# winddori2002/DEX-TTS

Hardware: AMD Instinct MI355X
Metric: mel-frames/s at n_timesteps=50, 80-ch mel (sampler only); RTF (higher is better)
Workload: dtype bf16; 1 GPU; gedex_b1: gedex_lj B=1/GPU T=512 n_timesteps=50 (BASELINE.json configs[1]); global_batch=1, frames=512, hipgraph=False, parallelism=1 GPU

## Files before the change

### dex_tts_amd/csrc/conv3x3_bf16.hip

```cpp
#include "kernels.h"
#include <cstdlib>
#include <cstdio>
#include "lp_util.h"
#include "kernels_lp.h"
#include "conv_gn.h"

namespace dex {
namespace DEX_LP_NS {

typedef float f32x16 __attribute__((ext_vector_type(16)));
typedef unsigned short u16;
typedef unsigned u32x4 __attribute__((ext_vector_type(4)));

__device__ __forceinline__ float cv_mish(float x) {
    const float e = __expf(fminf(x, 20.f));
    const float n = e * (e + 2.f);
    return x * (n * __builtin_amdgcn_rcpf(n + 2.f));
}

template <int NT, int COUT>
__device__ __forceinline__ void cv_epilogue(const Conv3P& p, f32x16 (&acc)[NT], int b, int ho, int w0, int nbase, int lane, int tid,
                                            long long* gnred) {
    const int i = lane & 31, hh = lane >> 5;
    constexpr int cpg = COUT / 8;
    if (p.gn_stats) { if (tid < 16) gnred[tid] = 0; __syncthreads(); }
    const bool full = ho < p.H && w0 + 32 <= p.W;
    const long ybase = (long)b * p.H * p.W * COUT + ((long)ho * p.W + w0 + 4 * hh) * COUT + nbase + i;
    float* yl = p.Y + ybase;
    u16* yh = reinterpret_cast<u16*>(p.Y) + ybase;
    const bool yb = p.y_bf16 != 0;
#pragma unroll
    for (int t = 0; t < NT; ++t) {
        const int n = nbase + t * 32 + i;
        const float bias = p.bias[n];
        float gs = 0.f, gss = 0.f;
        if (full && yb) {
            const bool odd = (lane & 1) != 0;
            u16* yp = yh + (odd ? 16 * COUT - 1 : 0) + t * 32;
#pragma unroll
            for (int r = 0; r < 16; ++r) { const float v = acc[t][r] + bias; gs += v; gss = fmaf(v, v, gss); }
#pragma unroll
            for (int j = 0; j < 8; ++j) {
                const float lo_r = acc[t][j] + bias, hi_r = acc[t][8 + j] + bias;
                const float recv = lane_xor1(odd ? lo_r : hi_r);
                const float mine = odd ? hi_r : lo_r;
                const unsigned pk = odd ? pack2_lp(recv, mine) : pack2_lp(mine, recv);
                *reinterpret_cast<unsigned*>(yp + ((j & 3) + 8 * (j >> 2)) * COUT) = pk;
            }
        } else if (full) {
            const bool odd = (lane & 1) != 0;
            float* yp = yl + (odd ? 16 * COUT - 1 : 0) + t * 32;
#pragma unroll
            for (int r = 0; r < 16; ++r) { const float v = acc[t][r] + bias; gs += v; gss = fmaf(v, v, gss); }
#pragma unroll
            for (int j = 0; j < 8; ++j) {
                const float lo_r = acc[t][j] + bias, hi_r = acc[t][8 + j] + bias;
                const float recv = lane_xor1(odd ? lo_r : hi_r);
                const float mine = odd ? hi_r : lo_r;
                *reinterpret_cast<float2*>(yp + ((j & 3) + 8 * (j >> 2)) * COUT) = odd ? make_float2(recv, mine) : make_float2(mine, recv);
            }
        } else {
#pragma unroll
            for (int r = 0; r < 16; ++r) {
                const int wo = w0 + (r & 3) + 8 * (r >> 2) + 4 * hh;
                const bool ok = ho < p.H && wo < p.W;
                const float v = acc[t][r] + bias;
                const float vs = ok ? v : 0.f;
                gs += vs; gss = fmaf(vs, vs, gss);
                if (ok) {
                    if (yb) yh[((r & 3) + 8 * (r >> 2)) * COUT + t * 32] = lp_bits(v);
                    else yl[((r & 3) + 8 * (r >> 2)) * COUT + t * 32] = v;
                }
            }
        }
        if (p.gn_stats) {
            for (int o = 1; o < cpg; o <<= 1) { gs += __shfl_xor(gs, o); gss += __shfl_xor(gss, o); }
            gs += __shfl_xor(gs, 32); gss += __shfl_xor(gss, 32);
            if (hh == 0 && (i & (cpg - 1)) == 0) {
                const double inv_n = 1.0 / ((double)p.H * p.W * cpg);
                gn_add(&gnred[(n / cpg) * 2], gn_fix(gs, inv_n)); gn_add(&gnred[(n / cpg) * 2 + 1], gn_fix(gss, inv_n));
            }
        }
    }
    if (p.gn_stats) {
        __syncthreads();
        if (tid < 16) {
            const long long v = gnred[tid];
            if (v != 0) {
                const int slot = (blockIdx.x + blockIdx.y * gridDim.x) % GN_SLOTS;
                gn_add(p.gn_stats + (((long)b * 8 + (tid >> 1)) * GN_SLOTS + slot) * 2 + (tid & 1), v);
            }
        }
    }
}

template <int NT, int COUT>
__device__ __forceinline__ void cv_res_store(const Conv3P& p, const f32x16 (&accr)[NT], int b, int ho, int w0, int nb, int lane) {
    const int i = lane & 31, hh = lane >> 5;
    float* yl = p.res_y + ((long)b * p.H * p.W + (long)ho * p.W + w0 + 4 * hh) * COUT + nb + i;
    const bool rfull = ho < p.H && w0 + 32 <= p.W;
    const bool odd = (lane & 1) != 0;
#pragma unroll
    for (int t = 0; t < NT; ++t) {
        const float bias = p.res_b[nb + t * 32 + i];
        if (rfull) {
            float* yp = yl + (odd ? 16 * COUT - 1 : 0) + t * 32;
#pragma unroll
            for (int j = 0; j < 8; ++j) {
                const float lo_r = accr[t][j] + bias, hi_r = accr[t][8 + j] + bias;
                const float recv = lane_xor1(odd ? lo_r : hi_r);
                const float mine = odd ? hi_r : lo_r;
                *reinterpret_cast<float2*>(yp + ((j & 3) + 8 * (j >> 2)) * COUT) = odd ? make_float2(recv, mine) : make_float2(mine, recv);
            }
        } else {
#pragma unroll
            for (int r = 0; r < 16; ++r) {
                const int wo = w0 + (r & 3) + 8 * (r >> 2) + 4 * hh;
                if (ho < p.H && wo < p.W) yl[((r & 3) + 8 * (r >> 2)) * COUT + t * 32] = accr[t][r] + bias;
            }
        }
    }
}

template <int CC, int COUT, int NSL, int TH, bool PRO2 = false, bool RES = false, bool XB = false, int NW = 4>
__global__ __launch_bounds__(64 * NW) void conv3x3_lp_kernel(const Conv3P p) {
    constexpr int PW = 34, PH = TH + 2;
    constexpr int LDP = CC + 8;
    constexpr int WN = NW / TH;
    constexpr int NTHR = 64 * NW;
    constexpr int NT = NSL / 32 / WN;
    constexpr int NSLICE = COUT / NSL;
    constexpr int ITEMS = PH * PW * (CC / 8);
    constexpr int NI = (ITEMS + NTHR - 1) / NTHR;
    constexpr int WITEMS = NSL * CC / 8;
    constexpr int WPT = (WITEMS + NTHR - 1) / NTHR;
    constexpr bool WFULL = WITEMS % NTHR == 0;
    constexpr int RING = CC == 128 ? (PRO2 ? 1 : 2) : 3;
    constexpr int NPASS = TH == 5 ? (CC == 128 ? (PRO2 ? 6 : 3) : (PRO2 ? 3 : XB ? 1 : 2))
                                  : CC == 128 ? (TH == 8 ? (PRO2 ? 8 : 4) : (PRO2 ? 5 : 2)) : (PRO2 ? 3 : 1);
    constexpr int NIP = (NI + NPASS - 1) / NPASS;
#ifdef DEX_LP_WSPLIT
    constexpr int NTAP = 18;
#else
    constexpr int NTAP = 9;
#endif
    static_assert(NT >= 1 && WPT >= 1 && NW % TH == 0 && NTHR % (CC / 8) == 0, "tile");
    extern __shared__ __attribute__((aligned(16))) u16 smem[];
    u16* patch = smem;
    u16* wbuf = smem + PH * PW * LDP;
    u16* rbuf = wbuf + 2 * NSL * LDP;
    __shared__ long long gnred[16];
    constexpr int COEF_N = (TH == 8) ? 128 : 256;
    __shared__ __attribute__((aligned(16))) float coef[3][COEF_N];

    const int tid = threadIdx.x, lane = tid & 63, wave = tid >> 6;
    const int i = lane & 31, hh = lane >> 5;
    const int wrow = wave % TH, wcol = wave / TH;
#ifdef DEX_TIMING
    long long tk[8] = {0, 0, 0, 0, 0, 0, 0, 0};
    const long long tk0 = __builtin_readcyclecounter();
    long long tlast = tk0;
#define CSTAMP(k) do { const long long now_ = __builtin_readcyclecounter(); tk[k] += now_ - tlast; tlast = now_; } while (0)
#else
#define CSTAMP(k) do {} while (0)
#endif
    const int xs = p.skip_dead ? (int)((blockIdx.x + blockIdx.y + blockIdx.z) % gridDim.x) : (int)blockIdx.x;
    const int w0 = xs * 32, h0 = blockIdx.y * TH;
    const int b = blockIdx.z / NSLICE, slice = blockIdx.z % NSLICE;
    const int step = p.step + b * p.row_bstride;
    const float* X = p.X + (long)b * p.H * p.W * p.ldx + p.x_coff;
    const u16* Xh = reinterpret_cast<const u16*>(p.X) + (long)b * p.H * p.W * p.ldx + p.x_coff;
    const float* mrow = p.mask + (long)b * p.mask_bstride;
    const int K = 9 * p.Cin;
    const u16* Wg = reinterpret_cast<const u16*>(p.Wbf) + (long)slice * NSL * K;
    const bool pro = p.pro_stats != nullptr;
    if constexpr (!PRO2) {
        if (p.skip_dead) {
            const int wi = w0 - 1 + (lane < 34 ? lane : 33);
            const float mv = (unsigned)wi < (unsigned)p.W ? mrow[wi * p.mask_ws] : 0.f;
            if (__builtin_amdgcn_ballot_w64(mv != 0.f) == 0) {
                f32x16 zacc[NT];
#pragma unroll
                for (int t = 0; t < NT; ++t)
#pragma unroll
                    for (int r = 0; r < 16; ++r) zacc[t][r] = 0.f;
                if constexpr (RES) cv_res_store<NT, COUT>(p, zacc, b, h0 + wrow, w0, slice * NSL + wcol * NT * 32, lane);
                cv_epilogue<NT, COUT>(p, zacc, b, h0 + wrow, w0, slice * NSL + wcol * NT * 32, lane, tid, gnred);
                return;
            }
        }
    }

    f32x16 acc[NT];
#pragma unroll
    for (int t = 0; t < NT; ++t)
#pragma unroll
        for (int r = 0; r < 16; ++r) acc[t][r] = 0.f;

    f32x16 accr[RES ? NT : 1];
    if constexpr (RES) {
#pragma unroll
        for (int t = 0; t < NT; ++t)
#pragma unroll
            for (int r = 0; r < 16; ++r) accr[t][r] = 0.f;
    }
    int wofs[WPT], wlds[WPT];
    bool wok[WPT];
#pragma unroll
    for (int j = 0; j < WPT; ++j) {
        const int it = tid + NTHR * j;
        const int n = it / (CC / 8), c8 = (it % (CC / 8)) * 8;
        wofs[j] = n * K + c8;
        wlds[j] = n * LDP + c8;
        wok[j] = WFULL || it < WITEMS;
    }
    const int pc8 = (tid % (CC / 8)) * 8;

    CvGnLoads gnl{};
    if (pro) gnl = cv_gn_issue(p, b, tid, step);
    const int nchunk = p.Cin / CC;
    for (int ch = 0; ch < nchunk; ++ch) {
        const int cbase = ch * CC;
        u32x4 w0r[WPT], wr[RING][WPT], rwr[RES ? WPT : 1];
#ifdef DEX_LP_WSPLIT
        u32x4 rwl[RES ? WPT : 1];
#define WS_TAPOFS(t) ((long)((t) % 9) * p.Cin + ((t) >= 9 ? p.w_lo_off : 0L))
#else
#define WS_TAPOFS(t) ((long)(t) * p.Cin)
#endif
        float4 sc0, sc1, sh0, sh1, t0, t1;
#pragma unroll
        for (int ps = 0; ps < NPASS; ++ps) {
            float4 pf0[NIP], pf1[XB ? 1 : NIP], rf0[PRO2 ? NIP : 1], rf1[PRO2 ? NIP : 1];
            float pmk[NIP];
            bool pin[NIP];
#pragma unroll
            for (int q = 0; q < NIP; ++q) {
                const int it = min(tid + NTHR * (ps * NIP + q), ITEMS - 1);
                const int px = it / (CC / 8);
                const int pw = px % PW, ph = px / PW;
                const int hi = h0 + ph - 1, wi = w0 + pw - 1;
                const bool inb = (unsigned)hi < (unsigned)p.H && (unsigned)wi < (unsigned)p.W;
                const int hc = inb ? hi : 0, wc = inb ? wi : 0;
                if constexpr (XB) {
                    pf0[q] = *reinterpret_cast<const float4*>(Xh + ((long)hc * p.W + wc) * p.ldx + cbase + pc8);
                } else {
                    const float* src = X + ((long)hc * p.W + wc) * p.ldx + cbase + pc8;
                    pf0[q] = *reinterpret_cast<const float4*>(src);
                    pf1[q] = *reinterpret_cast<const float4*>(src + 4);
                }
                if constexpr (PRO2) {
                    const float* rs = p.pro_res + ((long)b * p.H * p.W + (long)hc * p.W + wc) * p.Cin + cbase + pc8;
                    rf0[q] = *reinterpret_cast<const float4*>(rs);
                    rf1[q] = *reinterpret_cast<const float4*>(rs + 4);
                }
                const float mk = mrow[wc * p.mask_ws];
                pmk[q] = inb ? mk : 0.f;
                pin[q] = inb;
            }
            if (ps == 0) {
                if constexpr (RES) {
                    const u16* Rg = reinterpret_cast<const u16*>(p.res_w) + (long)slice * NSL * p.Cin;
#pragma unroll
                    for (int j = 0; j < WPT; ++j) {
                        const int it = tid + NTHR * j;
                        if (!wok[j]) continue;
                        rwr[j] = *reinterpret_cast<const u32x4*>(Rg + (long)(it / (CC / 8)) * p.Cin + cbase + (it % (CC / 8)) * 8);
#ifdef DEX_LP_WSPLIT
                        rwl[j] = *reinterpret_cast<const u32x4*>(Rg + p.res_lo_off + (long)(it / (CC / 8)) * p.Cin + cbase + (it % (CC / 8)) * 8);
#endif
                    }
                }
#pragma unroll
                for (int j = 0; j < WPT; ++j) if (wok[j]) w0r[j] = *reinterpret_cast<const u32x4*>(Wg + wofs[j] + cbase);
#pragma unroll
                for (int s = 0; s < RING; ++s)
#pragma unroll
                    for (int j = 0; j < WPT; ++j) if (wok[j]) wr[s][j] = *reinterpret_cast<const u32x4*>(Wg + wofs[j] + WS_TAPOFS(s + 1) + cbase);
                CSTAMP(0);
                if (pro && ch == 0) cv_gn_finish<COEF_N>(p, gnl, tid, coef);
                __builtin_amdgcn_sched_barrier(0);
                lds_barrier();
                CSTAMP(1);
                if (pro) {
                    const int c = cbase + pc8;
                    sc0 = *reinterpret_cast<const float4*>(&coef[0][c]); sc1 = *reinterpret_cast<const float4*>(&coef[0][c + 4]);
                    sh0 = *reinterpret_cast<const float4*>(&coef[1][c]); sh1 = *reinterpret_cast<const float4*>(&coef[1][c + 4]);
                    t0 = *reinterpret_cast<const float4*>(&coef[2][c]); t1 = *reinterpret_cast<const float4*>(&coef[2][c + 4]);
                }
            }
#pragma unroll
            for (int q = 0; q < NIP; ++q) {
                float4 f0, f1;
                if constexpr (XB) {
                    const float4 r = pf0[q];
                    const unsigned u0 = __float_as_uint(r.x), u1 = __float_as_uint(r.y), u2 = __float_as_uint(r.z), u3 = __float_as_uint(r.w);
                    f0 = make_float4(lp_lo(u0), lp_hi(u0), lp_lo(u1), lp_hi(u1));
                    f1 = make_float4(lp_lo(u2), lp_hi(u2), lp_lo(u3), lp_hi(u3));
                } else { f0 = pf0[q]; f1 = pf1[q]; }
#ifdef DEX_SCALAR_PROLOGUE
                if (pro) {
                    f0.x = cv_mish(fmaf(f0.x, sc0.x, sh0.x)) + t0.x; f0.y = cv_mish(fmaf(f0.y, sc0.y, sh0.y)) + t0.y;
                    f0.z = cv_mish(fmaf(f0.z, sc0.z, sh0.z)) + t0.z; f0.w = cv_mish(fmaf(f0.w, sc0.w, sh0.w)) + t0.w;
                    f1.x = cv_mish(fmaf(f1.x, sc1.x, sh1.x)) + t1.x; f1.y = cv_mish(fmaf(f1.y, sc1.y, sh1.y)) + t1.y;
                    f1.z = cv_mish(fmaf(f1.z, sc1.z, sh1.z)) + t1.z; f1.w = cv_mish(fmaf(f1.w, sc1.w, sh1.w)) + t1.w;
                }
#else
                if (pro) {
                    const f32x2 a0 = mish2_add(f32x2{f0.x, f0.y} * f32x2{sc0.x, sc0.y} + f32x2{sh0.x, sh0.y}, f32x2{t0.x, t0.y});
                    const f32x2 a1 = mish2_add(f32x2{f0.z, f0.w} * f32x2{sc0.z, sc0.w} + f32x2{sh0.z, sh0.w}, f32x2{t0.z, t0.w});
                    const f32x2 a2 = mish2_add(f32x2{f1.x, f1.y} * f32x2{sc1.x, sc1.y} + f32x2{sh1.x, sh1.y}, f32x2{t1.x, t1.y});
                    const f32x2 a3 = mish2_add(f32x2{f1.z, f1.w} * f32x2{sc1.z, sc1.w} + f32x2{sh1.z, sh1.w}, f32x2{t1.z, t1.w});
                    f0 = make_float4(a0.x, a0.y, a1.x, a1.y); f1 = make_float4(a2.x, a2.y, a3.x, a3.y);
                }
#endif
                const float mk = pmk[q];
                const int it = tid + NTHR * (ps * NIP + q);
                if constexpr (PRO2) {
                    f0.x = fmaf(f0.x, mk, rf0[q].x); f0.y = fmaf(f0.y, mk, rf0[q].y); f0.z = fmaf(f0.z, mk, rf0[q].z); f0.w = fmaf(f0.w, mk, rf0[q].w);
                    f1.x = fmaf(f1.x, mk, rf1[q].x); f1.y = fmaf(f1.y, mk, rf1[q].y); f1.z = fmaf(f1.z, mk, rf1[q].z); f1.w = fmaf(f1.w, mk, rf1[q].w);
                    const int px_ = it / (CC / 8), pw_ = px_ % PW, ph_ = px_ / PW;
                    if (slice == 0 && it < ITEMS && pin[q] && ph_ >= 1 && ph_ <= TH && pw_ >= 1 && pw_ <= 32) {
                        float* xo = p.pro_xout + ((long)b * p.H * p.W + (long)(h0 + ph_ - 1) * p.W + (w0 + pw_ - 1)) * p.Cin + cbase + pc8;
                        *reinterpret_cast<float4*>(xo) = f0;
                        *reinterpret_cast<float4*>(xo + 4) = f1;
                    }
                }
                uint4 v;
                v.x = pack2_lp(f0.x * mk, f0.y * mk); v.y = pack2_lp(f0.z * mk, f0.w * mk);
                v.z = pack2_lp(f1.x * mk, f1.y * mk); v.w = pack2_lp(f1.z * mk, f1.w * mk);
                if (it < ITEMS) *reinterpret_cast<uint4*>(patch + (it / (CC / 8)) * LDP + pc8) = v;
            }
        }
#pragma unroll
        for (int j = 0; j < WPT; ++j) if (wok[j]) *reinterpret_cast<u32x4*>(wbuf + wlds[j]) = w0r[j];
        if constexpr (RES) {
#pragma unroll
            for (int j = 0; j < WPT; ++j) if (wok[j]) *reinterpret_cast<u32x4*>(rbuf + wlds[j]) = rwr[j];
        }
        CSTAMP(2);
#pragma unroll
        for (int tt = 0; tt < NTAP; ++tt) {
            const int tap = tt % 9;
            lds_barrier();
            if (tt + 1 < NTAP) {
                u16* wn = wbuf + ((tt + 1) & 1) * NSL * LDP;
#pragma unroll
                for (int j = 0; j < WPT; ++j) if (wok[j]) *reinterpret_cast<u32x4*>(wn + wlds[j]) = wr[tt % RING][j];
                if (tt + 1 + RING < NTAP) {
#pragma unroll
                    for (int j = 0; j < WPT; ++j)
                        if (wok[j]) wr[tt % RING][j] = *reinterpret_cast<const u32x4*>(Wg + wofs[j] + WS_TAPOFS(tt + 1 + RING) + cbase);
                }
                __builtin_amdgcn_sched_barrier(0);
            }
#ifdef DEX_LP_WSPLIT
            if constexpr (RES) {
                if (tt == 5) {
#pragma unroll
                    for (int j = 0; j < WPT; ++j) if (wok[j]) *reinterpret_cast<u32x4*>(rbuf + wlds[j]) = rwl[j];
                }
            }
#endif
            const u16* wb = wbuf + (tt & 1) * NSL * LDP;
            const int kh = tap / 3, kw = tap - kh * 3;
            const u16* ap = patch + ((wrow + kh) * PW + i + kw) * LDP + hh * 8;
            const u16* bp = wb + (wcol * NT * 32 + i) * LDP + hh * 8;
#pragma unroll
            for (int ks = 0; ks < CC / 16; ++ks) {
                const lp8 af = *reinterpret_cast<const lp8*>(ap + ks * 16);
#pragma unroll
                for (int t = 0; t < NT; ++t) {
                    const lp8 bf = *reinterpret_cast<const lp8*>(bp + t * 32 * LDP + ks * 16);
                    acc[t] = DEX_MFMA_LP(af, bf, acc[t], 0, 0, 0);
                }
                if constexpr (RES) {
                    if (tap == 4) {
#pragma unroll
                        for (int t = 0; t < NT; ++t) {
                            const lp8 rf = *reinterpret_cast<const lp8*>(rbuf + (wcol * NT * 32 + t * 32 + i) * LDP + hh * 8 + ks * 16);
                            accr[t] = DEX_MFMA_LP(af, rf, accr[t], 0, 0, 0);
                        }
                    }
                }
            }
        }
    }
    if constexpr (RES) cv_res_store<NT, COUT>(p, accr, b, h0 + wrow, w0, slice * NSL + wcol * NT * 32, lane);
    CSTAMP(3);
    cv_epilogue<NT, COUT>(p, acc, b, h0 + wrow, w0, slice * NSL + wcol * NT * 32, lane, tid, gnred);
#ifdef DEX_TIMING
    CSTAMP(4);
    if (p.dbg && tid == 0) {
        long long* d = p.dbg + ((long)(blockIdx.z * gridDim.y + blockIdx.y) * gridDim.x + blockIdx.x) * 8;
        for (int k = 0; k < 5; ++k) d[k] = tk[k];
        unsigned hw, xcc;
        asm volatile("s_getreg_b32 %0, hwreg(HW_REG_HW_ID)" : "=s"(hw));
        asm volatile("s_getreg_b32 %0, hwreg(HW_REG_XCC_ID)" : "=s"(xcc));
        d[5] = hw; d[6] = xcc & 15u;
        d[7] = __builtin_readcyclecounter() - tk0;
    }
#endif
}

template <int CC, int COUT, int NSL, int TH, bool PRO2 = false, bool RES = false, bool XB = false, int NW = 4>
static void launch_c3(const Conv3P& p, hipStream_t st) {
    constexpr int LDP = CC + 8;
    const size_t lds = ((size_t)(TH + 2) * 34 * LDP + (2 + (RES ? 1 : 0)) * NSL * LDP) * sizeof(u16);
    static bool attr = false;
    if (!attr) {
        hipFuncSetAttribute(reinterpret_cast<const void*>(&conv3x3_lp_kernel<CC, COUT, NSL, TH, PRO2, RES, XB, NW>), hipFuncAttributeMaxDynamicSharedMemorySize, (int)lds);
        attr = true;
    }
    dim3 grid((p.W + 31) / 32, (p.H + TH - 1) / TH, p.B * (COUT / NSL));
    Conv3P q = p;
    q.skip_dead = (p.B >= 4 && (long)grid.x * grid.y * grid.z >= 1024 && knob_or("DEX_CONV_SKIP_DEAD", 1) != 0) ? 1 : 0;
    static char sym[96];
    if (!sym[0]) snprintf(sym, sizeof sym, "conv3x3_lp_kernel<%d,%d,%d,%d,%d,%d,%d,%d>", CC, COUT, NSL, TH, (int)PRO2, (int)RES, (int)XB, NW);
    g_last_symbol = sym;
    hipLaunchKernelGGL((conv3x3_lp_kernel<CC, COUT, NSL, TH, PRO2, RES, XB, NW>), grid, dim3(64 * NW), lds, st, q);
}

bool conv3x3_bf16_tail_supported(int C) {
#if defined(DEX_LP_WSPLIT) && !defined(DEX_WS_HAVE_CONV3)
    return false;
#endif
    return C == 64 || C == 128; }
bool conv3x3_bf16_xb_supported(int Cin, int Cout) {
#if defined(DEX_LP_WSPLIT) && !defined(DEX_WS_HAVE_CONV3)
    return false;
#endif
    return Cin == Cout && (Cin == 64 || Cin == 128); }
bool conv3x3_bf16_res_supported(int Cin, int Cout) {
#if defined(DEX_LP_WSPLIT) && !defined(DEX_WS_HAVE_CONV3_RES)
    return false;
#endif
    return (Cout == 128 && Cin == 64) || (Cout == 64 && (Cin == 128 || Cin == 256)); }
bool conv3x3_bf16_supported(int Cin, int Cout) {
#if defined(DEX_LP_WSPLIT) && !defined(DEX_WS_HAVE_CONV3)
    return false;
#endif
   
    return (Cin == 64 || Cin == 128 || Cin == 256) && (Cout == 64 || Cout == 128);
}

bool conv3x3_plain_lp_in_supported(int H, int W, int B, int Cin, int Cout) {
#if defined(DEX_LP_WSPLIT) && !defined(DEX_WS_HAVE_CONV3)
    return false;
#endif
   
    const int w8 = knob_or("DEX_CONV_W8", 1);
    const long tiles4 = (long)((W + 31) / 32) * ((H + 3) / 4) * B;
    return w8 && tiles4 >= 256 && Cin == 64 && Cout == 128;
}

bool conv3x3_cat_lp_in_supported(int H, int W, int B, int Cin, int Cout) {
#if defined(DEX_LP_WSPLIT) && !defined(DEX_WS_HAVE_CONV3_RES)
    return false;
#endif
   
    if (Cout != 64 || Cin < 128 || Cin % 128 != 0) return false;
    const int w8 = knob_or("DEX_CONV_W8", 1);
    const long small_max = knob_or("DEX_CONV_SMALL_MAX", 256);
    const long tiles4 = (long)((W + 31) / 32) * ((H + 3) / 4) * B;
    return w8 && tiles4 >= small_max;
}

static bool launch_c3_round1(const Conv3P& p, bool small, hipStream_t st) {
    if (!knob_or("DEX_CONV_ROUND1", 1)) return false;
    const bool tail_ = p.pro_res != nullptr;
#ifdef DEX_LP_WSPLIT
    const bool c64 = p.Cin == 64 && p.Cout == 64 && !p.res_w && !tail_;
#else
    const bool c64 = p.Cin == 64 && p.Cout == 64 && !p.res_w;
#endif
    const bool r128 = p.Cin == 64 && p.Cout == 128 && p.res_w && !tail_ && !p.x_bf16;
    if (!c64 && !r128) return false;
    const long strips = (long)((p.W + 31) / 32) * p.B;
    const long cur = c64 ? strips * (small ? (p.H + 1) / 2 : (p.H + 3) / 4) : strips * (small ? (p.H + 1) / 2 * 2 : (p.H + 3) / 4);
    const long one = strips * ((p.H + 4) / 5) * (c64 ? 1 : 4);
    const long ncu = device_cus();
    if (cur <= ncu || one > ncu || one * 4 < ncu * 3) return false;
    if (c64) {
#ifndef DEX_LP_WSPLIT
        if (tail_) { p.x_bf16 ? launch_c3<64, 64, 64, 5, true, false, true, 10>(p, st) : launch_c3<64, 64, 64, 5, true, false, false, 10>(p, st); return true; }
#endif
        p.x_bf16 ? launch_c3<64, 64, 64, 5, false, false, true, 10>(p, st) : launch_c3<64, 64, 64, 5, false, false, false, 10>(p, st);
    } else {
        launch_c3<64, 128, 32, 5, false, true, false, 5>(p, st);
    }
    return true;
}

void launch_conv3x3_lp(const Conv3P& p, hipStream_t st) {
    if (const int tpw = conv3x3_stream_tiles(p)) { launch_conv3x3_stream(p, tpw, st); return; }
    if (conv3x3_regw_form(p)) { launch_conv3x3_regw(p, st); return; }
    const bool tail_ = p.pro_res != nullptr;
    const long tiles4 = (long)((p.W + 31) / 32) * ((p.H + 3) / 4) * p.B;
    const long small_max = knob_or("DEX_CONV_SMALL_MAX", 256);
    const bool small = tiles4 < small_max;
    const int w8 = knob_or("DEX_CONV_W8", 1);
    const int th8 = knob_or("DEX_CONV_TH8", 1);
    if (th8 && w8 && !small && !tail_ && p.Cin == 128 && p.Cout == 128 && !p.res_w && p.H % 8 == 0 && (long)((p.W + 31) / 32) * (p.H / 8) * p.B >= 512) {
        p.x_bf16 ? launch_c3<128, 128, 128, 8, false, false, true, 8>(p, st) : launch_c3<128, 128, 128, 8, false, false, false, 8>(p, st);
        return;
    }
    if (w8 && !small && p.Cin == 128 && p.Cout == 128 && !p.res_w) {
        if (p.x_bf16) { tail_ ? launch_c3<128, 128, 128, 4, true, false, true, 8>(p, st) : launch_c3<128, 128, 128, 4, false, false, true, 8>(p, st); }
        else { tail_ ? launch_c3<128, 128, 128, 4, true, false, false, 8>(p, st) : launch_c3<128, 128, 128, 4, false, false, false, 8>(p, st); }
        return;
    }
    if (w8 && !small && p.res_w && p.Cout == 128 && p.Cin == 64) {
        p.x_bf16 ? launch_c3<64, 128, 128, 4, false, true, true, 8>(p, st) : launch_c3<64, 128, 128, 4, false, true, false, 8>(p, st);
        return;
    }
    if (th8 && w8 && !small && p.res_w && p.Cout == 64 && p.Cin >= 128 && !p.pro_stats && p.H % 8 == 0 && (long)((p.W + 31) / 32) * (p.H / 8) * p.B >= 512) {
        p.x_bf16 ? launch_c3<128, 64, 64, 8, false, true, true, 8>(p, st) : launch_c3<128, 64, 64, 8, false, true, false, 8>(p, st);
        return;
    }
    if (w8 && !small && p.res_w && p.Cout == 64 && p.Cin >= 128) {
        p.x_bf16 ? launch_c3<128, 64, 64, 4, false, true, true, 8>(p, st) : launch_c3<128, 64, 64, 4, false, true, false, 8>(p, st);
        return;
    }
    if (launch_c3_round1(p, small, st)) return;
    if (p.x_bf16) {
        if (tail_) {
            if (p.Cin == 64) { small ? launch_c3<64, 64, 64, 2, true, false, true>(p, st) : launch_c3<64, 64, 64, 4, true, false, true>(p, st); }
            else { small ? launch_c3<128, 128, 64, 2, true, false, true>(p, st) : launch_c3<128, 128, 128, 4, true, false, true>(p, st); }
        } else {
            if (p.Cin == 64) { small ? launch_c3<64, 64, 64, 2, false, false, true>(p, st) : launch_c3<64, 64, 64, 4, false, false, true>(p, st); }
            else { small ? launch_c3<128, 128, 64, 2, false, false, true>(p, st) : launch_c3<128, 128, 128, 4, false, false, true>(p, st); }
        }
        return;
    }
    if (tail_) {
        if (p.Cin == 64 && p.Cout == 64) { small ? launch_c3<64, 64, 64, 2, true>(p, st) : launch_c3<64, 64, 64, 4, true>(p, st); }
        else { small ? launch_c3<128, 128, 64, 2, true>(p, st) : launch_c3<128, 128, 128, 4, true>(p, st); }
        return;
    }
    if (p.res_w) {
        if (p.Cout == 128 && p.Cin == 64) { small ? launch_c3<64, 128, 64, 2, false, true>(p, st) : launch_c3<64, 128, 128, 4, false, true>(p, st); return; }
        if (p.Cout == 64 && p.Cin >= 128) { small ? launch_c3<128, 64, 64, 2, false, true>(p, st) : launch_c3<128, 64, 64, 4, false, true>(p, st); return; }
    }
    if (p.Cout == 64) {
        if (p.Cin == 64) { small ? launch_c3<64, 64, 64, 2>(p, st) : launch_c3<64, 64, 64, 4>(p, st); }
        else { small ? launch_c3<128, 64, 64, 2>(p, st) : launch_c3<128, 64, 64, 4>(p, st); }
    } else {
        if (p.Cin == 64) { small ? launch_c3<64, 128, 64, 2>(p, st) : launch_c3<64, 128, 128, 4>(p, st); }
        else { small ? launch_c3<128, 128, 64, 2>(p, st) : launch_c3<128, 128, 128, 4>(p, st); }
    }
}

}
}
```

### dex_tts_amd/csrc/dex_api.hip

```cpp
#include <hip/hip_runtime.h>
#include <cstdlib>

#include <cmath>
#include <cstdarg>
#include <atomic>
#include <cstdio>
#include <mutex>
#include <cstring>
#include <map>
#include <unordered_map>
#include <string_view>
#include <string>
#include <vector>

#include "../../include/dex_amd.h"
#include "kernels.h"
#include "weight_store.h"

using namespace dex;

namespace dex {
namespace {
const char* const KNOB_NAMES[] = {
    "DEX_CONV_STREAM", "DEX_CONV_PP", "DEX_CONV_SKIP_DEAD", "DEX_H_BF16", "DEX_ATTN_SEPARATE", "DEX_ATTN_Q64", "DEX_ATTN_Q64_TAIL", "DEX_ATTN_Q64_HALF", "DEX_DIT_XCDS", "DEX_ATTN_GENERIC", "DEX_RES2", "DEX_LP_INTER", "DEX_DIT_CHAIN",
    "DEX_DIT_CLUSTER", "DEX_DIT_CLUSTER_LOCAL", "DEX_ATTN_X_LP", "DEX_RES_X_LP", "DEX_CAT_LP", "DEX_XCD_MAP", "DEX_DEBUG_DROP_HANDOFF", "DEX_PATCH_FUSED",
    "DEX_CONV_DOWN", "DEX_CONVT_UP", "DEX_DEBUG_PLAN",
    "DEX_ATTN_SHARED_W8", "DEX_CONVT_MT", "DEX_CONVT_WGS", "DEX_CONV_DOWN_WGS", "DEX_CONV_REGW", "DEX_CONV_REGW_RES", "DEX_CONV_SMALL_MAX", "DEX_CONV_TH8",
    "DEX_CONV_W8", "DEX_DWCONV_CAP", "DEX_FINAL_CAP", "DEX_FIRST_CAP", "DEX_FIRST_MFMA", "DEX_GEMM_NWALK", "DEX_NWALK_SPLIT", "DEX_NWALK_BM", "DEX_POS_COL", "DEX_POS_COL_MIN",
    "DEX_POS_CT", "DEX_REGW_MIN_TILES", "DEX_REGW_WGS", "DEX_ROWCHAIN64", "DEX_ROWCHAIN64A", "DEX_TIV_CAP", "DEX_TV_CHAIN", "DEX_TIV_FOLD", "DEX_LINATTN_NSUB", "DEX_TV_FOLD", "DEX_OUT2_MIN", "DEX_NWALK_DMA",
    "DEX_LINATTN_HEADWAVES", "DEX_LINATTN_OUT2_HW", "DEX_CONV_ROUND1"};
constexpr int N_KNOBS = (int)(sizeof(KNOB_NAMES) / sizeof(KNOB_NAMES[0]));
int knob_parse(const char* e) {
    if (!e) return KNOB_UNSET;
    char* end = nullptr;
    const long v = strtol(e, &end, 10);
    if (end == e) {
        static bool warned = false;
        if (!warned) { warned = true; fprintf(stderr, "libdexamd: ignoring a DEX_* knob whose value '%s' is not an integer\n", e); }
        return KNOB_UNSET;
    }
    return (int)v;
}
struct KnobSnapshot {
    int v[N_KNOBS];
    KnobSnapshot() { for (int i = 0; i < N_KNOBS; ++i) v[i] = knob_parse(getenv(KNOB_NAMES[i])); }
};
thread_local const KnobSnapshot* t_knobs = nullptr;
struct WsplitScope {
    bool prev;
    explicit WsplitScope(bool on) : prev(g_lp_wsplit) { g_lp_wsplit = on; }
    ~WsplitScope() { g_lp_wsplit = prev; }
};
struct KnobScope {
    const KnobSnapshot* prev;
    explicit KnobScope(const KnobSnapshot* k) : prev(t_knobs) { t_knobs = k; }
    ~KnobScope() { t_knobs = prev; }
};
}
static int knob_index(const char* name) {
    static const std::unordered_map<std::string_view, int> idx = [] {
        std::unordered_map<std::string_view, int> m;
        for (int i = 0; i < N_KNOBS; ++i) m.emplace(KNOB_NAMES[i], i);
        return m;
    }();
    const auto it = idx.find(std::string_view(name));
    return it == idx.end() ? -1 : it->second;
}
int knob(const char* name) {
    if (t_knobs) {
        const int i = knob_index(name);
        if (i >= 0) return t_knobs->v[i];
    }
    return knob_parse(getenv(name));
}
}
static_assert(PREC_FP32 == DEX_PREC_FP32 && PREC_BF16 == DEX_PREC_BF16 && PREC_FP16 == DEX_PREC_FP16 && PREC_FP16X2 == DEX_PREC_FP16X2, "kernels.h mirrors DexPrecision");

namespace {
void xcd_map_probe();

struct TD { float* p; int ld; int coff; int C; int lp = 0; };

struct ResW { PackedW w1, w2, wr; const float *b1, *g1, *be1, *b2, *g2, *be2, *br, *mlp_w, *mlp_b; int cin, cout; };
constexpr int ATT_KSPLIT_MAX = 4;
static int att_split_cap(long tokens) { return tokens <= 20480 ? 8 : ATT_KSPLIT_MAX; }
static bool attention_q64_regime(int N, int B) {
    if (N < 1024) return dit_sep64_small_n(N, B) && dit_rowchain64_form(N, B, 0);
    const int ks = attention_q64_ksplit(N, B, att_split_cap((long)B * N));
    const int nt32 = (N + 31) / 32, ng = (nt32 + 7) / 8;
    return 2L * B * ng * ks >= 128;
}
struct LinW { PackedW wqkv; const float *wqkv_raw, *wout_raw, *bias_eff, *g; LpView wkv[3], wq_frag[3]; int C; };
struct DitBlockW { PackedW wqkv, wproj, wfc1, wfc2; const float *bqkv, *bproj, *bfc1, *bfc2, *ada_w, *ada_b; };

struct Prof { std::string name; hipEvent_t a, b; double flops, bytes; };
struct ProfAgg { std::string name; int calls; double ms, flops, bytes; };

struct Arena {
    char* base = nullptr; size_t off = 0, cap = 0; bool dry = true;
    void* take(size_t bytes) {
        off = (off + 255) & ~size_t(255);
        void* p = dry ? nullptr : (void*)(base + off);
        if (!dry && trace) fprintf(stderr, "plan[%d] off %zu bytes %zu\n", trace++, off, bytes);
        off += bytes;
        return p;
    }
    int trace = 0;
    float* f(size_t n) { return (float*)take(n * sizeof(float)); }
};

}

struct DexCtx : WeightStore {
    DexCtx() : WeightStore("") {}
    DexConfig cfg{};
    int lpi() const { return precision == DEX_PREC_FP16X2 ? 2 : precision == DEX_PREC_FP16 ? 1 : 0; }
    int lp_kind() const { return precision == DEX_PREC_BF16 ? 1 : 2; }
    bool lp() const { return precision != DEX_PREC_FP32; }
    bool tuned = true;
    int precision = DEX_PREC_FP32;
    std::vector<std::vector<ResW>> down_res, up_res;
    std::vector<LinW> down_lin, up_lin;
    std::vector<PackedW> down_ds_w;
    std::vector<std::vector<PackedW>> up_us_w;
    std::vector<const float*> down_ds_b, up_us_b;
    const float *fc_w3 = nullptr, *fc_w1 = nullptr;
    PackedW fin_w, pe_pw, fl_w, tv_wk, tv_wv, tv_wl;
    PackedW pos_w;
    const float *fin_b = nullptr, *fin_g = nullptr, *fin_be = nullptr, *fconv_w = nullptr, *fconv_b = nullptr;
    const float *pe_dw = nullptr, *pe_db = nullptr, *pe_pb = nullptr, *pos_b = nullptr, *freq_pos = nullptr;
    std::vector<DitBlockW> blocks;
    const float *fl_b = nullptr, *fl_ada_w = nullptr, *fl_ada_b = nullptr;
    const float *tv_wq_raw = nullptr;
    float *mel_basis = nullptr, *mel_filt = nullptr; void* mel_ws = nullptr; size_t mel_ws_bytes = 0;
    const int* last_xerr = nullptr;
    int* st_host = nullptr; hipEvent_t st_ev = nullptr; bool st_pending = false;
    struct Tap { std::string name; const float* p; std::vector<int64_t> shape; };
    std::vector<Tap> taps;
    bool prof_on = false;
    std::vector<Prof> prof;
    std::vector<ProfAgg> prof_agg;
    struct GraphEntry { std::vector<uint64_t> key; hipGraphExec_t exec; uint64_t stamp; const int* xerr; };
    std::vector<GraphEntry> graphs;
    uint64_t graph_clock = 0;
    void drop_graphs() { for (auto& g : graphs) hipGraphExecDestroy(g.exec); graphs.clear(); }
    template <typename F> int replay(const std::vector<uint64_t>& key, hipStream_t st, F&& enqueue);
    void reset_records() {
        taps.clear();
        if (prof_on) { for (auto& pr : prof) { hipEventDestroy(pr.a); hipEventDestroy(pr.b); } prof.clear(); prof_agg.clear(); }
    }
};

template <typename F> int DexCtx::replay(const std::vector<uint64_t>& key, hipStream_t st, F&& enqueue) {
    GraphEntry* hit = nullptr;
    for (auto& g : graphs) if (g.key == key) { hit = &g; break; }
    if (!hit) {
        constexpr size_t MAX_GRAPHS = 8;
        if (graphs.size() >= MAX_GRAPHS) {
            size_t lru = 0;
            for (size_t i = 1; i < graphs.size(); ++i) if (graphs[i].stamp < graphs[lru].stamp) lru = i;
            hipGraphExecDestroy(graphs[lru].exec);
            graphs.erase(graphs.begin() + lru);
        }
        hipGraph_t graph = nullptr;
        DEX_HIPCHK(this, hipStreamBeginCapture(st, hipStreamCaptureModeThreadLocal));
        const int rc = enqueue();
        hipError_t ec = hipStreamEndCapture(st, &graph);
        if (rc) { if (graph) hipGraphDestroy(graph); return rc; }
        if (ec != hipSuccess || !graph) return fail(DEX_ERR_HIP, "stream capture failed: %s", hipGetErrorString(ec));
        hipGraphExec_t exec = nullptr;
        ec = hipGraphInstantiate(&exec, graph, nullptr, nullptr, 0);
        hipGraphDestroy(graph);
        if (ec != hipSuccess) return fail(DEX_ERR_HIP, "hipGraphInstantiate failed: %s", hipGetErrorString(ec));
        graphs.push_back({key, exec, 0, last_xerr});
        hit = &graphs.back();
    }
    last_xerr = hit->xerr;
    hit->stamp = ++graph_clock;
    DEX_HIPCHK(this, hipGraphLaunch(hit->exec, st));
    DEX_HIPCHK(this, hipGetLastError());
    return DEX_OK;
}

namespace {

int stage_dim(const DexConfig& c, int i) { return c.dim * c.dim_mults[i]; }
int in_planes(const DexConfig& c) { return 2 + (c.n_spks > 1 ? 1 : 0); }
int mid_dim(const DexConfig& c) { return stage_dim(c, c.n_stages - 1); }
int mid_h(const DexConfig& c) { return c.n_feats >> (c.n_stages - 1); }
int grid_h(const DexConfig& c) { return mid_h(c) / c.dit_stride; }
int token_rows(const DexConfig& c) { return (mid_h(c) + 2 * (c.dit_patch / 2) - c.dit_patch) / c.dit_stride + 1; }
int token_cols(const DexConfig& c, int wmid) {
    const int p = c.dit_patch, s = c.dit_stride;
    const int wp = (wmid % p == 0) ? wmid : wmid + (p - wmid % p);
    return (wp + 2 * (p / 2) - p) / s + 1;
}
int mlp_hidden(const DexConfig& c) { return (int)(c.dit_hidden * c.dit_mlp_ratio); }

void add_resnet(DexCtx* x, const std::string& p, int cin, int cout, int tdim) {
    x->add(p + ".mlp.1.weight", {cout, tdim}); x->add(p + ".mlp.1.bias", {cout});
    for (int blk = 1; blk <= 2; ++blk) {
        const std::string q = p + ".block" + std::to_string(blk) + ".block";
        x->add(q + ".0.weight", {cout, blk == 1 ? cin : cout, 3, 3}); x->add(q + ".0.bias", {cout});
        x->add(q + ".1.weight", {cout}); x->add(q + ".1.bias", {cout});
    }
    if (cin != cout) { x->add(p + ".res_conv.weight", {cout, cin, 1, 1}); x->add(p + ".res_conv.bias", {cout}); }
}
void add_linattn(DexCtx* x, const std::string& p, int c) {
    x->add(p + ".fn.g", {1});
    x->add(p + ".fn.fn.to_qkv.weight", {384, c, 1, 1});
    x->add(p + ".fn.fn.to_out.weight", {c, 128, 1, 1});
    x->add(p + ".fn.fn.to_out.bias", {c});
}
void build_inventory(DexCtx* x) {
    const DexConfig& c = x->cfg;
    const int d = c.dim;
    x->add("mlp.0.weight", {4 * d, d}); x->add("mlp.0.bias", {4 * d});
    x->add("mlp.2.weight", {d, 4 * d}); x->add("mlp.2.bias", {d});
    if (c.variant == DEX_VARIANT_DEX)
        for (const char* n : {"mlp_adap", "mlp_adap_sty"}) {
            const std::string s(n);
            x->add(s + ".0.weight", {d, d}); x->add(s + ".0.bias", {d});
            x->add(s + ".2.weight", {2 * d, d}); x->add(s + ".2.bias", {2 * d});
        }
    if (c.n_spks > 1) {
        const int e = c.spk_emb_dim;
        x->add("spk_mlp.0.weight", {4 * e, e}); x->add("spk_mlp.0.bias", {4 * e});
        x->add("spk_mlp.2.weight", {c.n_feats, 4 * e}); x->add("spk_mlp.2.bias", {c.n_feats});
    }
    for (int i = 0; i < c.n_stages; ++i) {
        const int ci = i == 0 ? in_planes(c) : stage_dim(c, i - 1), co = stage_dim(c, i);
        const std::string p = "downs." + std::to_string(i);
        add_resnet(x, p + ".0", ci, co, d); add_resnet(x, p + ".1", co, co, d); add_linattn(x, p + ".2", co);
        if (i < c.n_stages - 1) { x->add(p + ".3.conv.weight", {co, co, 3, 3}); x->add(p + ".3.conv.bias", {co}); }
    }
    const int hid = c.dit_hidden, mid = mid_dim(c), mh = mlp_hidden(c);
    x->add("vit.freq_new_pos_embed", {1, hid, grid_h(c), 1});
    x->add("vit.x_embedder.proj.0.weight", {mid, 1, c.dit_patch, c.dit_patch}); x->add("vit.x_embedder.proj.0.bias", {mid});
    x->add("vit.x_embedder.proj.2.weight", {hid, mid, 1, 1}); x->add("vit.x_embedder.proj.2.bias", {hid});
    x->add("vit.t_embedder.mlp.0.weight", {hid, 256}); x->add("vit.t_embedder.mlp.0.bias", {hid});
    x->add("vit.t_embedder.mlp.2.weight", {hid, hid}); x->add("vit.t_embedder.mlp.2.bias", {hid});
    x->add("vit.pos_conv.0.weight", {hid, hid / c.dit_conv_pos_groups, c.dit_conv_pos, c.dit_conv_pos});
    x->add("vit.pos_conv.0.bias", {hid});
    for (int k = 0; k < c.dit_depth; ++k) {
        const std::string p = "vit.blocks." + std::to_string(k);
        x->add(p + ".attn.qkv.weight", {3 * hid, hid}); x->add(p + ".attn.qkv.bias", {3 * hid});
        x->add(p + ".attn.proj.weight", {hid, hid}); x->add(p + ".attn.proj.bias", {hid});
        x->add(p + ".mlp.fc1.weight", {mh, hid}); x->add(p + ".mlp.fc1.bias", {mh});
        x->add(p + ".mlp.fc2.weight", {hid, mh}); x->add(p + ".mlp.fc2.bias", {hid});
        x->add(p + ".adaLN_modulation.1.weight", {6 * hid, hid}); x->add(p + ".adaLN_modulation.1.bias", {6 * hid});
    }
    const int so = c.dit_stride * c.dit_stride * mid;
    x->add("vit.final_layer.linear.weight", {so, hid}); x->add("vit.final_layer.linear.bias", {so});
    x->add("vit.final_layer.adaLN_modulation.1.weight", {2 * hid, hid}); x->add("vit.final_layer.adaLN_modulation.1.bias", {2 * hid});
    if (c.variant == DEX_VARIANT_DEX) {
        for (const char* w : {"w_q", "w_k", "w_v", "linear"}) x->add(std::string("tv_adaptor.") + w + ".weight", {mid, mid});
        for (const char* s : {"mean_sap", "std_sap"}) {
            x->add(std::string("tiv_adaptor.") + s + ".W.weight", {1, mid});
            x->add(std::string("tiv_adaptor.") + s + ".W.bias", {1});
        }
    }
    for (int j = 0; j < c.n_stages - 1; ++j) {
        const int i = c.n_stages - 1 - j;
        const int ci = stage_dim(c, i - 1), co = stage_dim(c, i);
        const std::string p = "ups." + std::to_string(j);
        add_resnet(x, p + ".0", co * 2, ci, d); add_resnet(x, p + ".1", ci, ci, d); add_linattn(x, p + ".2", ci);
        x->add(p + ".3.conv.weight", {ci, ci, 4, 4}); x->add(p + ".3.conv.bias", {ci});
    }
    x->add("final_block.block.0.weight", {d, d, 3, 3}); x->add("final_block.block.0.bias", {d});
    x->add("final_block.block.1.weight", {d}); x->add("final_block.block.1.bias", {d});
    x->add("final_conv.weight", {1, d, 1, 1}); x->add("final_conv.bias", {1});
}

__global__ void pack_convt_kernel(const float* src, float* dst, int Cin, int Cout) {
    const long total = 4L * 4 * Cin * Cout;
    for (long i = (long)blockIdx.x * blockDim.x + threadIdx.x; i < total; i += (long)gridDim.x * blockDim.x) {
        const int co = (int)(i % Cout);
        const int ci = (int)((i / Cout) % Cin);
        const int tap = (int)((i / ((long)Cout * Cin)) % 4);
        const int par = (int)(i / ((long)Cout * Cin * 4));
        const int ph = par >> 1, pw = par & 1, th = tap >> 1, tw = tap & 1;
        const int kh = (ph ? 0 : 1) + 2 * th, kw = (pw ? 0 : 1) + 2 * tw;
        dst[i] = src[(((long)ci * Cout + co) * 4 + kh) * 4 + kw];
    }
}

}

extern "C" {

const char* dex_version(void) { return "dexamd 0.1 (gfx950)"; }

int dex_ctx_create(const DexConfig* cfg, DexCtx** out) {
    if (!cfg || !out) return DEX_ERR_ARG;
    DexCtx* x = new DexCtx();
    x->cfg = *cfg;
    const DexConfig& c = x->cfg;
    *out = x;
    if (c.n_feats != 80) return x->fail(DEX_ERR_ARG, "n_feats must be 80 (diffusion.py:226 hard-codes it)");
    if (c.n_stages < 2 || c.n_stages > 4) return x->fail(DEX_ERR_ARG, "n_stages must be in [2,4]");
    if (c.dim != 64 && c.dim != 128) return x->fail(DEX_ERR_ARG, "dim must be 64 (GeDEX, DEX-VCTK/ESD) or 128 (DEX-LibriTTS)");
    if (c.dit_heads < 1 || c.dit_hidden % c.dit_heads || !attention_head_dim_supported(c.dit_hidden / c.dit_heads))
        return x->fail(DEX_ERR_ARG, "DiT head_dim must be 64, 128, 192 or 256 (hidden %d heads %d)", c.dit_hidden, c.dit_heads);
    if (c.dit_hidden % 64 || c.dit_hidden > 512) return x->fail(DEX_ERR_ARG, "dit_hidden must be a multiple of 64, <= 512");
    if (mlp_hidden(c) % 64) return x->fail(DEX_ERR_ARG, "mlp hidden must be a multiple of 64");
    if (c.dit_conv_pos_groups < 1 || c.dit_hidden % c.dit_conv_pos_groups || (c.dit_hidden / c.dit_conv_pos_groups) % 16 ||
        c.dit_hidden / c.dit_conv_pos_groups > 64)
        return x->fail(DEX_ERR_ARG, "pos-conv groups must be 16, 32, 48 or 64 channels wide");
    if (c.dit_conv_pos % 2) return x->fail(DEX_ERR_ARG, "conv_pos must be even");
    if (c.variant == DEX_VARIANT_DEX && !attention_head_dim_supported(mid_dim(c)))
        return x->fail(DEX_ERR_ARG, "DEX adaptors need mid_dim 64, 128, 192 or 256 (the cross-attention's head_dim)");
    x->tuned = c.dim == 64 && c.dit_hidden == 256 && c.dit_heads == 2 && c.dit_hidden / c.dit_conv_pos_groups == 32 &&
               (c.variant != DEX_VARIANT_DEX || mid_dim(c) == 128);
    build_inventory(x);
    xcd_map_probe();
    return DEX_OK;
}

void dex_ctx_destroy(DexCtx* x) {
    if (!x) return;
    x->release();
    if (x->mel_basis) hipFree(x->mel_basis);
    if (x->mel_filt) hipFree(x->mel_filt);
    if (x->mel_ws) hipFree(x->mel_ws);
    x->drop_graphs();
    for (auto& pr : x->prof) { hipEventDestroy(pr.a); hipEventDestroy(pr.b); }
    if (x->st_ev) hipEventDestroy(x->st_ev);
    if (x->st_host) hipHostFree(x->st_host);
    delete x;
}

const char* dex_last_error(const DexCtx* x) { return x ? x->err.c_str() : "null context"; }
int dex_ctx_num_weights(const DexCtx* x) { return x ? (int)x->keys.size() : 0; }
// ... 1606 lines not shown
```

Measured before the change: 28240 mel-frames/s.

## Add resident-weight conv3x3 schedule loading all nine taps into LDS once

Adds an RW template variant of the bf16 conv3x3 kernel that loads all nine weight taps for a single 64-channel input chunk into LDS, interleaved with the patch loads in a single pass. The MFMA loop then runs over all taps and k-steps with a double-buffered register pipeline, in place of the rotating per-tap weight ring with its per-tap barriers. It is enabled by default through a new DEX_CONV_RESIDENT knob for the round-1 Cin=64 paths and for small-grid 64->64 convs. The aim is to cut per-tap synchronisation and weight-staging latency, at the cost of much larger LDS use per block, which may lower occupancy.

After: 28790 mel-frames/s (median of 6 runs). 1.02x the previous value.

```diff
diff --git a/dex_tts_amd/csrc/conv3x3_bf16.hip b/dex_tts_amd/csrc/conv3x3_bf16.hip
--- a/dex_tts_amd/csrc/conv3x3_bf16.hip
+++ b/dex_tts_amd/csrc/conv3x3_bf16.hip
@@ -122,7 +122,7 @@
     }
 }
 
-template <int CC, int COUT, int NSL, int TH, bool PRO2 = false, bool RES = false, bool XB = false, int NW = 4>
+template <int CC, int COUT, int NSL, int TH, bool PRO2 = false, bool RES = false, bool XB = false, int NW = 4, bool RW = false>
 __global__ __launch_bounds__(64 * NW) void conv3x3_lp_kernel(const Conv3P p) {
     constexpr int PW = 34, PH = TH + 2;
     constexpr int LDP = CC + 8;
@@ -136,19 +136,24 @@
     constexpr int WPT = (WITEMS + NTHR - 1) / NTHR;
     constexpr bool WFULL = WITEMS % NTHR == 0;
     constexpr int RING = CC == 128 ? (PRO2 ? 1 : 2) : 3;
-    constexpr int NPASS = TH == 5 ? (CC == 128 ? (PRO2 ? 6 : 3) : (PRO2 ? 3 : XB ? 1 : 2))
+    constexpr int NPASS = RW ? 1
+                        : TH == 5 ? (CC == 128 ? (PRO2 ? 6 : 3) : (PRO2 ? 3 : XB ? 1 : 2))
                                   : CC == 128 ? (TH == 8 ? (PRO2 ? 8 : 4) : (PRO2 ? 5 : 2)) : (PRO2 ? 3 : 1);
     constexpr int NIP = (NI + NPASS - 1) / NPASS;
+    constexpr int RWI = 9 * WITEMS;
+    constexpr int RWPT = (RWI + NTHR - 1) / NTHR;
+    constexpr int RWB = (RWPT + NPASS - 1) / NPASS;
 #ifdef DEX_LP_WSPLIT
     constexpr int NTAP = 18;
 #else
     constexpr int NTAP = 9;
 #endif
     static_assert(NT >= 1 && WPT >= 1 && NW % TH == 0 && NTHR % (CC / 8) == 0, "tile");
+    static_assert(!RW || NTAP == 9, "the resident schedule holds nine taps");
     extern __shared__ __attribute__((aligned(16))) u16 smem[];
     u16* patch = smem;
     u16* wbuf = smem + PH * PW * LDP;
-    u16* rbuf = wbuf + 2 * NSL * LDP;
+    u16* rbuf = wbuf + (RW ? 9 : 2) * NSL * LDP;
     __shared__ long long gnred[16];
     constexpr int COEF_N = (TH == 8) ? 128 : 256;
     __shared__ __attribute__((aligned(16))) float coef[3][COEF_N];
@@ -218,7 +223,7 @@
 
     CvGnLoads gnl{};
     if (pro) gnl = cv_gn_issue(p, b, tid, step);
-    const int nchunk = p.Cin / CC;
+    const int nchunk = RW ? 1 : p.Cin / CC;
     for (int ch = 0; ch < nchunk; ++ch) {
         const int cbase = ch * CC;
         u32x4 w0r[WPT], wr[RING][WPT], rwr[RES ? WPT : 1];
@@ -258,6 +263,17 @@
                 pmk[q] = inb ? mk : 0.f;
                 pin[q] = inb;
             }
+            u32x4 rwv[RW ? RWB : 1];
+            if constexpr (RW) {
+#pragma unroll
+                for (int j = 0; j < RWB; ++j) {
+                    const int it = tid + NTHR * (ps * RWB + j);
+                    if (ps * RWB + j < RWPT && (RWI % NTHR == 0 || it < RWI)) {
+                        const int r = it % WITEMS;
+                        rwv[j] = *reinterpret_cast<const u32x4*>(Wg + (r / (CC / 8)) * K + (it / WITEMS) * p.Cin + (r % (CC / 8)) * 8);
+                    }
+                }
+            }
             if (ps == 0) {
                 if constexpr (RES) {
                     const u16* Rg = reinterpret_cast<const u16*>(p.res_w) + (long)slice * NSL * p.Cin;
@@ -271,16 +287,18 @@
 #endif
                     }
                 }
-#pragma unroll
-                for (int j = 0; j < WPT; ++j) if (wok[j]) w0r[j] = *reinterpret_cast<const u32x4*>(Wg + wofs[j] + cbase);
-#pragma unroll
-                for (int s = 0; s < RING; ++s)
-#pragma unroll
-                    for (int j = 0; j < WPT; ++j) if (wok[j]) wr[s][j] = *reinterpret_cast<const u32x4*>(Wg + wofs[j] + WS_TAPOFS(s + 1) + cbase);
+                if constexpr (!RW) {
+#pragma unroll
+                    for (int j = 0; j < WPT; ++j) if (wok[j]) w0r[j] = *reinterpret_cast<const u32x4*>(Wg + wofs[j] + cbase);
+#pragma unroll
+                    for (int s = 0; s < RING; ++s)
+#pragma unroll
+                        for (int j = 0; j < WPT; ++j) if (wok[j]) wr[s][j] = *reinterpret_cast<const u32x4*>(Wg + wofs[j] + WS_TAPOFS(s + 1) + cbase);
+                }
                 CSTAMP(0);
                 if (pro && ch == 0) cv_gn_finish<COEF_N>(p, gnl, tid, coef);
                 __builtin_amdgcn_sched_barrier(0);
-                lds_barrier();
+                if (!RW || pro) lds_barrier();
                 CSTAMP(1);
                 if (pro) {
                     const int c = cbase + pc8;
@@ -331,14 +349,62 @@
                 v.z = pack2_lp(f1.x * mk, f1.y * mk); v.w = pack2_lp(f1.z * mk, f1.w * mk);
                 if (it < ITEMS) *reinterpret_cast<uint4*>(patch + (it / (CC / 8)) * LDP + pc8) = v;
             }
-        }
-#pragma unroll
-        for (int j = 0; j < WPT; ++j) if (wok[j]) *reinterpret_cast<u32x4*>(wbuf + wlds[j]) = w0r[j];
+            if constexpr (RW) {
+#pragma unroll
+                for (int j = 0; j < RWB; ++j) {
+                    const int it = tid + NTHR * (ps * RWB + j);
+                    if (ps * RWB + j < RWPT && (RWI % NTHR == 0 || it < RWI)) {
+                        const int r = it % WITEMS;
+                        *reinterpret_cast<u32x4*>(wbuf + ((it / WITEMS) * NSL + r / (CC / 8)) * LDP + (r % (CC / 8)) * 8) = rwv[j];
+                    }
+                }
+            }
+        }
+        if constexpr (!RW) {
+#pragma unroll
+            for (int j = 0; j < WPT; ++j) if (wok[j]) *reinterpret_cast<u32x4*>(wbuf + wlds[j]) = w0r[j];
+        }
         if constexpr (RES) {
 #pragma unroll
             for (int j = 0; j < WPT; ++j) if (wok[j]) *reinterpret_cast<u32x4*>(rbuf + wlds[j]) = rwr[j];
         }
         CSTAMP(2);
+        if constexpr (RW) {
+            lds_barrier();
+            constexpr int KS = CC / 16;
+            const u16* ap = patch + (wrow * PW + i) * LDP + hh * 8;
+            const u16* bp = wbuf + (wcol * NT * 32 + i) * LDP + hh * 8;
+            const u16* rp = rbuf + (wcol * NT * 32 + i) * LDP + hh * 8;
+            lp8 af[2], bf[2][NT], rf[2][RES ? NT : 1];
+            af[0] = *reinterpret_cast<const lp8*>(ap);
+#pragma unroll
+            for (int t = 0; t < NT; ++t) bf[0][t] = *reinterpret_cast<const lp8*>(bp + t * 32 * LDP);
+#pragma unroll
+            for (int s = 0; s < 9 * KS; ++s) {
+                if (s + 1 < 9 * KS) {
+                    const int tap = (s + 1) / KS, ks = (s + 1) % KS, kh = tap / 3, kw = tap - kh * 3;
+                    af[(s + 1) & 1] = *reinterpret_cast<const lp8*>(ap + (kh * PW + kw) * LDP + ks * 16);
+#pragma unroll
+                    for (int t = 0; t < NT; ++t) bf[(s + 1) & 1][t] = *reinterpret_cast<const lp8*>(bp + (tap * NSL + t * 32) * LDP + ks * 16);
+                    if constexpr (RES) {
+                        if (tap == 4) {
+#pragma unroll
+                            for (int t = 0; t < NT; ++t) rf[(s + 1) & 1][t] = *reinterpret_cast<const lp8*>(rp + t * 32 * LDP + ks * 16);
+                        }
+                    }
+                }
+                __builtin_amdgcn_sched_barrier(0);
+#pragma unroll
+                for (int t = 0; t < NT; ++t) acc[t] = DEX_MFMA_LP(af[s & 1], bf[s & 1][t], acc[t], 0, 0, 0);
+                if constexpr (RES) {
+                    if (s / KS == 4) {
+#pragma unroll
+                        for (int t = 0; t < NT; ++t) accr[t] = DEX_MFMA_LP(af[s & 1], rf[s & 1][t], accr[t], 0, 0, 0);
+                    }
+                }
+                __builtin_amdgcn_sched_barrier(0);
+            }
+        } else {
 #pragma unroll
         for (int tt = 0; tt < NTAP; ++tt) {
             const int tap = tt % 9;
@@ -384,6 +450,7 @@
                     }
                 }
             }
+        }
         }
     }
     if constexpr (RES) cv_res_store<NT, COUT>(p, accr, b, h0 + wrow, w0, slice * NSL + wcol * NT * 32, lane);
@@ -403,22 +470,23 @@
 #endif
 }
 
-template <int CC, int COUT, int NSL, int TH, bool PRO2 = false, bool RES = false, bool XB = false, int NW = 4>
+template <int CC, int COUT, int NSL, int TH, bool PRO2 = false, bool RES = false, bool XB = false, int NW = 4, bool RW = false>
 static void launch_c3(const Conv3P& p, hipStream_t st) {
     constexpr int LDP = CC + 8;
-    const size_t lds = ((size_t)(TH + 2) * 34 * LDP + (2 + (RES ? 1 : 0)) * NSL * LDP) * sizeof(u16);
+    const size_t lds = ((size_t)(TH + 2) * 34 * LDP + ((RW ? 9 : 2) + (RES ? 1 : 0)) * NSL * LDP) * sizeof(u16);
     static bool attr = false;
     if (!attr) {
-        hipFuncSetAttribute(reinterpret_cast<const void*>(&conv3x3_lp_kernel<CC, COUT, NSL, TH, PRO2, RES, XB, NW>), hipFuncAttributeMaxDynamicSharedMemorySize, (int)lds);
+        hipFuncSetAttribute(reinterpret_cast<const void*>(&conv3x3_lp_kernel<CC, COUT, NSL, TH, PRO2, RES, XB, NW, RW>), hipFuncAttributeMaxDynamicSharedMemorySize, (int)lds);
         attr = true;
     }
     dim3 grid((p.W + 31) / 32, (p.H + TH - 1) / TH, p.B * (COUT / NSL));
+    if (RW && p.Cin != CC) { fprintf(stderr, "libdexamd: resident conv3x3 form needs Cin == %d in one chunk (got %d)\n", CC, p.Cin); abort(); }
     Conv3P q = p;
     q.skip_dead = (p.B >= 4 && (long)grid.x * grid.y * grid.z >= 1024 && knob_or("DEX_CONV_SKIP_DEAD", 1) != 0) ? 1 : 0;
     static char sym[96];
-    if (!sym[0]) snprintf(sym, sizeof sym, "conv3x3_lp_kernel<%d,%d,%d,%d,%d,%d,%d,%d>", CC, COUT, NSL, TH, (int)PRO2, (int)RES, (int)XB, NW);
+    if (!sym[0]) snprintf(sym, sizeof sym, "conv3x3_lp_kernel<%d,%d,%d,%d,%d,%d,%d,%d%s>", CC, COUT, NSL, TH, (int)PRO2, (int)RES, (int)XB, NW, RW ? ",resident" : "");
     g_last_symbol = sym;
-    hipLaunchKernelGGL((conv3x3_lp_kernel<CC, COUT, NSL, TH, PRO2, RES, XB, NW>), grid, dim3(64 * NW), lds, st, q);
+    hipLaunchKernelGGL((conv3x3_lp_kernel<CC, COUT, NSL, TH, PRO2, RES, XB, NW, RW>), grid, dim3(64 * NW), lds, st, q);
 }
 
 bool conv3x3_bf16_tail_supported(int C) {
@@ -465,6 +533,8 @@
     const long tiles4 = (long)((W + 31) / 32) * ((H + 3) / 4) * B;
     return w8 && tiles4 >= small_max;
 }
+
+static bool conv3x3_resident_on() { return knob_or("DEX_CONV_RESIDENT", 1) != 0; }
 
 static bool launch_c3_round1(const Conv3P& p, bool small, hipStream_t st) {
     if (!knob_or("DEX_CONV_ROUND1", 1)) return false;
@@ -481,6 +551,15 @@
     const long one = strips * ((p.H + 4) / 5) * (c64 ? 1 : 4);
     const long ncu = device_cus();
     if (cur <= ncu || one > ncu || one * 4 < ncu * 3) return false;
+#ifndef DEX_LP_WSPLIT
+    if (conv3x3_resident_on()) {
+        if (c64 && !tail_) {
+            p.x_bf16 ? launch_c3<64, 64, 64, 5, false, false, true, 10, true>(p, st) : launch_c3<64, 64, 64, 5, false, false, false, 10, true>(p, st);
+            return true;
+        }
+        if (!c64) { launch_c3<64, 128, 32, 5, false, true, false, 5, true>(p, st); return true; }
+    }
+#endif
     if (c64) {
 #ifndef DEX_LP_WSPLIT
         if (tail_) { p.x_bf16 ? launch_c3<64, 64, 64, 5, true, false, true, 10>(p, st) : launch_c3<64, 64, 64, 5, true, false, false, 10>(p, st); return true; }
@@ -490,6 +569,19 @@
         launch_c3<64, 128, 32, 5, false, true, false, 5>(p, st);
     }
     return true;
+}
+
+static bool launch_c3_small_resident(const Conv3P& p, bool small, hipStream_t st) {
+#ifdef DEX_LP_WSPLIT
+    return false;
+#else
+    if (!small || !conv3x3_resident_on() || p.Cin != 64 || p.Cout != 64 || p.res_w) return false;
+    if ((long)((p.W + 31) / 32) * ((p.H + 1) / 2) * p.B > device_cus()) return false;
+    const bool tail_ = p.pro_res != nullptr;
+    if (tail_) { p.x_bf16 ? launch_c3<64, 64, 64, 2, true, false, true, 4, true>(p, st) : launch_c3<64, 64, 64, 2, true, false, false, 4, true>(p, st); }
+    else { p.x_bf16 ? launch_c3<64, 64, 64, 2, false, false, true, 4, true>(p, st) : launch_c3<64, 64, 64, 2, false, false, false, 4, true>(p, st); }
+    return true;
+#endif
 }
 
 void launch_conv3x3_lp(const Conv3P& p, hipStream_t st) {
@@ -523,6 +615,7 @@
         return;
     }
     if (launch_c3_round1(p, small, st)) return;
+    if (launch_c3_small_resident(p, small, st)) return;
     if (p.x_bf16) {
         if (tail_) {
             if (p.Cin == 64) { small ? launch_c3<64, 64, 64, 2, true, false, true>(p, st) : launch_c3<64, 64, 64, 4, true, false, true>(p, st); }
diff --git a/dex_tts_amd/csrc/dex_api.hip b/dex_tts_amd/csrc/dex_api.hip
--- a/dex_tts_amd/csrc/dex_api.hip
+++ b/dex_tts_amd/csrc/dex_api.hip
@@ -28,7 +28,7 @@
     "DEX_ATTN_SHARED_W8", "DEX_CONVT_MT", "DEX_CONVT_WGS", "DEX_CONV_DOWN_WGS", "DEX_CONV_REGW", "DEX_CONV_REGW_RES", "DEX_CONV_SMALL_MAX", "DEX_CONV_TH8",
     "DEX_CONV_W8", "DEX_DWCONV_CAP", "DEX_FINAL_CAP", "DEX_FIRST_CAP", "DEX_FIRST_MFMA", "DEX_GEMM_NWALK", "DEX_NWALK_SPLIT", "DEX_NWALK_BM", "DEX_POS_COL", "DEX_POS_COL_MIN",
     "DEX_POS_CT", "DEX_REGW_MIN_TILES", "DEX_REGW_WGS", "DEX_ROWCHAIN64", "DEX_ROWCHAIN64A", "DEX_TIV_CAP", "DEX_TV_CHAIN", "DEX_TIV_FOLD", "DEX_LINATTN_NSUB", "DEX_TV_FOLD", "DEX_OUT2_MIN", "DEX_NWALK_DMA",
-    "DEX_LINATTN_HEADWAVES", "DEX_LINATTN_OUT2_HW", "DEX_CONV_ROUND1"};
+    "DEX_LINATTN_HEADWAVES", "DEX_LINATTN_OUT2_HW", "DEX_CONV_ROUND1", "DEX_CONV_RESIDENT"};
 constexpr int N_KNOBS = (int)(sizeof(KNOB_NAMES) / sizeof(KNOB_NAMES[0]));
 int knob_parse(const char* e) {
     if (!e) return KNOB_UNSET;
```
